# alessiodevoto/peekvit

Hardware: AMD Instinct MI355X
Metric: images/sec ViT-B/16 fwd @ batch 2048, 224x224 (higher is better)
Workload: dtype f16; 1 GPU; vit_b_16 forward, batch 2048/GPU, 224x224; global_batch=2048, parallelism=replicas x1 (batch-sharded, no collective), precision_mode=auto, streams=1, operands=IEEE fp16 operands, fp32 accumulate (same MFMA rate as bf16), range-guarded, range_guard_fallbacks=0

## Files before the change

peekvit_amd/_build.py:

```python
from __future__ import annotations

import glob
import os
import subprocess
import sys

HERE = os.path.dirname(os.path.abspath(__file__))
CSRC = os.path.join(HERE, "csrc")
LIB = os.path.join(HERE, "libpeekvit_hip.so")
LIB_F16 = os.path.join(HERE, "libpeekvit_hip_f16.so")
HIPCC = os.environ.get("HIPCC", "/opt/rocm/bin/hipcc")
FLAGS = ["--offload-arch=gfx950", "-O3", "-std=c++17", "-fPIC", "-Wno-unused-result"]
HEADERS = ("peekvit_hip.h", "peekvit_hip_moe.h", "peekvit_hip_ee.h", "peekvit_hip_sparse.h", "peekvit_hip_pct.h",
           "peekvit_hip_pct_train.h", "peekvit_hip_attn_stream.h", "peekvit_hip_pct_block.h", "peekvit_hip_rank_train.h", "peekvit_hip_rank_infer.h",
           "peekvit_hip_avit_train.h", "peekvit_hip_sparse_train.h", "peekvit_hip_avit_pack_train.h", "peekvit_hip_dropout.h", "peekvit_hip_sparse_long.h",
           "peekvit_hip_sparse_long_train.h", "peekvit_hip_avit_long.h")
FILE_FLAGS = {"pv_attention.hip": ["-mllvm", "-amdgpu-mfma-vgpr-form=1"], "pv_rowops.hip": ["-fno-slp-vectorize"],
              "pv_attention_stream.hip": ["-mllvm", "-amdgpu-mfma-vgpr-form=1"],
              "pv_ee.hip": ["-fno-slp-vectorize"],
              "pv_sparse.hip": ["-fno-slp-vectorize"],
              "pv_sparse_long.hip": ["-fno-slp-vectorize"],
              "pv_pct.hip": ["-fno-slp-vectorize"],
              "pv_pct_train.hip": ["-fno-slp-vectorize"],
              "pv_rank_train.hip": ["-fno-slp-vectorize"],
              "pv_avit_train.hip": ["-fno-slp-vectorize"],
              "pv_avit_pack_train.hip": ["-fno-slp-vectorize"],
              "pv_avit_long.hip": ["-fno-slp-vectorize"],
              "pv_dropout.hip": ["-fno-slp-vectorize"],
              "pv_sparse_train.hip": ["-fno-slp-vectorize", "-mllvm", "-amdgpu-mfma-vgpr-form=1"],
              "pv_sparse_long_train.hip": ["-fno-slp-vectorize"]}


def sources():
    return sorted(glob.glob(os.path.join(CSRC, "*.hip")))


def _stale() -> bool:
    if not os.path.exists(LIB) or not os.path.exists(LIB_F16):
        return True
    t = min(os.path.getmtime(LIB), os.path.getmtime(LIB_F16))
    deps = sources() + glob.glob(os.path.join(CSRC, "*.h")) + [os.path.join(os.path.dirname(HERE), "include", h) for h in HEADERS] + [os.path.abspath(__file__)]
    return any(os.path.getmtime(d) > t for d in deps)


def build(force: bool = False, verbose: bool = False) -> str:
    if not force and not _stale():
        return LIB
    procs = []
    variants = [("build", [], LIB), ("build_f16", ["-DPV_OPERAND_F16"], LIB_F16)]
# ... 49 lines not shown
```

peekvit_amd/_lib.py:

```python
from __future__ import annotations

import ctypes as C
import os
import threading

import torch

from ._build import LIB

_i64, _f32, _p, _i32 = C.c_int64, C.c_float, C.c_void_p, C.c_int32

PV_EPI_BIAS_BF16, PV_EPI_BIAS_GELU_BF16, PV_EPI_BIAS_RES_F32, PV_EPI_BIAS_POS_F32 = 0, 1, 2, 3
PV_EPI_BIAS_F32, PV_EPI_BIAS_GELU_SPLIT_BF16 = 4, 5
PV_EPI_BIAS_GELU_PAIR_BF16, PV_EPI_GELU_GRAD_BF16 = 6, 7
PV_WS_TRANSPOSE_COLSUM, PV_WS_COLSUM, PV_WS_LAYERNORM_BWD, PV_WS_GEMM_COLSUM_PARTIAL, PV_WS_GEMM_SPLITK = 1, 2, 3, 4, 5


class GemmArgs(C.Structure):
    _fields_ = [("struct_size", C.c_uint64), ("A", _p), ("W", _p), ("bias", _p), ("out", _p), ("res", _p), ("row_scale", _p), ("pos", _p),
                ("M", _i64), ("N", _i64), ("K", _i64), ("lda", _i64), ("ldw", _i64), ("ldo", _i64), ("ldr", _i64),
                ("rows_per_img_in", _i64), ("rows_per_img_out", _i64), ("row_off", _i64), ("qcols", _i64),
                ("qscale", _f32), ("epilogue", _i32),
                ("ln_gamma", _p), ("ln_beta", _p), ("ln_row_scale", _p), ("ln_out", _p), ("ln_eps", _f32),
                ("ksplit", _i32), ("colsum_partial", _p),
# ... 136 lines not shown

SIGNATURES_AVIT_PACK_TRAIN = {
    "pv_avit_pack_step_train": (C.c_int, [_p] * 4 + [_i64] * 4 + [_p] * 12 + [_i64, _p, _f32, _f32, _f32, C.c_int] + [_p] * 11),
    "pv_avit_pack_step_bwd": (C.c_int, [_p] * 16 + [_i64] * 6 + [_f32, C.c_int, _p]),
}

_u64 = C.c_uint64
SIGNATURES_DROPOUT = {
    "pv_dropout_keep_u8": (C.c_int, [_p, _u64, _u64, _i64, _i64, _f32, _p]),
    "pv_dropout_f32": (C.c_int, [_p, _p, _u64, _u64, _i64, _i64, _f32, _p]),
    "pv_dropout_residual": (C.c_int, [_p, _p, _p, _u64, _u64, _i64, _i64, _f32, _p]),
    "pv_dropout_bwd16": (C.c_int, [_p, _p, _u64, _u64, _i64, _i64, _f32, _p]),
    "pv_attention_stream_lse_drop_bf16": (C.c_int, [_p, _p, _p, _i64, _i64, _i64, _i64, _f32, _u64, _u64, _p, _p]),
    "pv_attention_stream_bwd16_drop_bf16": (C.c_int, [_p, _p, _p, _p, _p, _p, _p, _i64, _i64, _i64, _i64, _f32, _f32, _u64, _u64, _p]),
}

SIGNATURES_SPARSE_LONG = {
    "pv_attention_varlen_w_stream_bf16": SIGNATURES_SPARSE["pv_attention_varlen_w_bf16"],
    "pv_residual_pack_step_long": SIGNATURES_SPARSE["pv_residual_pack_step"],
}

SIGNATURES_SPARSE_LONG_TRAIN = {
    "pv_attention_varlen_w_stream_lse_bf16": SIGNATURES_SPARSE_TRAIN["pv_attention_varlen_w_lse_bf16"],
    "pv_attention_varlen_w_stream_bwd16_bf16": SIGNATURES_SPARSE_TRAIN["pv_attention_varlen_w_bwd16_bf16"],
    "pv_residual_pack_step_long_train": SIGNATURES_SPARSE_TRAIN["pv_residual_pack_step_train"],
    "pv_residual_pack_step_long_bwd": SIGNATURES_SPARSE_TRAIN["pv_residual_pack_step_bwd"],
}

SIGNATURES_AVIT_LONG = {
    "pv_avit_pack_step_long": SIGNATURES_AVIT_PACK_TRAIN["pv_avit_pack_step_train"],
    "pv_avit_pack_step_long_bwd": SIGNATURES_AVIT_PACK_TRAIN["pv_avit_pack_step_bwd"],
}

ABI_VERSION = 10
_lock = threading.Lock()
_libs: dict = {}

_OPERAND_DEFAULT = "bf16"
_tls = threading.local()
LIB_F16 = os.path.join(os.path.dirname(os.path.abspath(__file__)), "libpeekvit_hip_f16.so")


def current_operand() -> str:
    return getattr(_tls, "operand", _OPERAND_DEFAULT)


def set_operand(op: str) -> str:
    old = current_operand()
    _tls.operand = op
    return old


def __getattr__(name):
    if name == "OPERAND":
        return current_operand()
    raise AttributeError(f"module {__name__!r} has no attribute {name!r}")


def operand_dtype():
    import torch as _t
    return _t.float16 if current_operand() == "f16" else _t.bfloat16


class PeekvitHipError(RuntimeError):
    pass


def lib_path(operand: str = "bf16") -> str:
    return LIB_F16 if operand == "f16" else LIB


def load(operand=None):
    op = current_operand() if operand is None else operand
    lib = _libs.get(op)
    if lib is not None:
        return lib
    with _lock:
        lib = _libs.get(op)
        if lib is not None:
            return lib
        path = lib_path(op)
        if not os.path.exists(path):
            raise PeekvitHipError(
                f"{path} not found: the MI355X kernels are not built. Run `python -m peekvit_amd._build` "
                "(or __graft_entry__.build()); there is no fallback path.")
        lib = C.CDLL(path)
        for name, (res, args) in {**SIGNATURES, **SIGNATURES_MOE, **SIGNATURES_EE, **SIGNATURES_SPARSE, **SIGNATURES_PCT,
                                   **SIGNATURES_PCT_TRAIN, **SIGNATURES_ATTN_STREAM, **SIGNATURES_PCT_BLOCK, **SIGNATURES_RANK_TRAIN,
                                   **SIGNATURES_RANK_INFER, **SIGNATURES_AVIT_TRAIN, **SIGNATURES_SPARSE_TRAIN, **SIGNATURES_AVIT_PACK_TRAIN,
                                   **SIGNATURES_DROPOUT, **SIGNATURES_SPARSE_LONG, **SIGNATURES_SPARSE_LONG_TRAIN,
                                   **SIGNATURES_AVIT_LONG}.items():
            fn = getattr(lib, name)
            fn.restype, fn.argtypes = res, args
        if lib.pv_version() != ABI_VERSION:
            raise PeekvitHipError(f"{path} has ABI v{lib.pv_version()}, this package binds v{ABI_VERSION}: rebuild (python -m peekvit_amd._build)")
        if lib.pv_gemm_args_size() != C.sizeof(GemmArgs):
            raise PeekvitHipError(f"{path}: pv_gemm_args is {lib.pv_gemm_args_size()} bytes in the library, {C.sizeof(GemmArgs)} in this binding")
        if lib.pv_operand_type() != (1 if op == "f16" else 0):
            raise PeekvitHipError(f"{path} was built for a different operand type")
        _libs[op] = lib
    return lib


def check(code: int, what: str = "") -> None:
    if code != 0:
        msg = load().pv_error_string(code).decode()
        raise PeekvitHipError(f"{what}: {msg} (code {code})" if what else f"{msg} (code {code})")
```

peekvit_amd/csrc/pv_gemm.hip:

```cpp
#include "pv_rows.h"
#include "../../include/peekvit_hip_moe.h"
#include "pv_gelu_table.h"
#include <type_traits>
#include <cstdlib>

typedef __attribute__((ext_vector_type(8))) short s16x8;

#ifndef PV_STORE_NT
#define PV_STORE_NT 3
#endif
#define PV_STORE16(ptr, val) do { if (PV_STORE_NT & 1) __builtin_nontemporal_store((val), (ptr)); else *(ptr) = (val); } while (0)
#define PV_STORE32(ptr, val) do { if (PV_STORE_NT & 2) __builtin_nontemporal_store((val), (ptr)); else *(ptr) = (val); } while (0)
#ifndef PV_PF_MODE
#define PV_PF_MODE 2
#endif
#ifndef PV_EPI_PIPE
#define PV_EPI_PIPE 1
#endif

__device__ __forceinline__ float pv_fma_s(float a, float b, float c) {
    float r;
    asm("v_fma_f32 %0, %1, %2, %3" : "=v"(r) : "v"(a), "v"(b), "v"(c));
    return r;
}
__device__ __forceinline__ float pv_mul_s(float a, float b) {
    float r;
    asm("v_mul_f32 %0, %1, %2" : "=v"(r) : "v"(a), "v"(b));
    return r;
}
__device__ __forceinline__ float pv_gelu_poly(float x, const f32x4 c) {
    const pv_f32x2_t c02 = {c[0], c[1]}, c13 = {c[2], c[3]}, xx = {x, x};
    const pv_f32x2_t r = __builtin_elementwise_fma(c13, xx, c02);
    return pv_fma_s(x, pv_mul_s(x, r[1]), r[0]);
}
// ... 477 lines not shown
    if (row_off + Np > S || M > 0x7fffffff || B * S > 0x7fffffff) return PV_ERR_INVALID_ARG;
    GemmDev p = {};
    p.W = W; p.bias = bias; p.out = tokens; p.pos = pos;
    p.M = (int)M; p.N = (int)D; p.K = (int)(C * P * P);
    p.ldw = p.K; p.ldo = D;
    p.rpi = (int)Np; p.rpo = (int)S; p.row_off = (int)row_off;
    p.qscale = 1.0f;
    p.tiles_m = (int)((M + G1_BM - 1) / G1_BM); p.tiles_n = (int)((D + G1_BN - 1) / G1_BN);
    p.range_flag = range_flag;
    const PatchGeom gm = {img, (int)C, (int)R, (int)P, (int)Wp, (int)Np};
    static PvPerDevice attr_set;
    const int lds = 2 * 2 * G1_TILE_BYTES;
    if (attr_set.first_use()) (void)hipFuncSetAttribute(reinterpret_cast<const void*>(pv_patch_embed_kernel), hipFuncAttributeMaxDynamicSharedMemorySize, lds);
    PV_LAUNCH(pv_patch_embed_kernel, dim3((unsigned)(p.tiles_m * p.tiles_n)), dim3(256), lds, (hipStream_t)stream, p, gm);
    return pv_check_launch();
}

template <int EPI>
static int pv_launch_gemm128(const GemmDev& p, hipStream_t stream) {
    static PvPerDevice attr_set;
    const int lds = 2 * 2 * G1_TILE_BYTES;
    if (attr_set.first_use()) {
        (void)hipFuncSetAttribute(reinterpret_cast<const void*>(pv_gemm128_kernel<EPI>), hipFuncAttributeMaxDynamicSharedMemorySize, lds);
    }
    PV_LAUNCH(pv_gemm128_kernel<EPI>, dim3((unsigned)(p.tiles_m * p.tiles_n * (p.ksplit > 1 ? p.ksplit : 1))), dim3(256), lds, stream, p);
    return pv_check_launch();
}

constexpr int G2_BM = 256, G2_BN = 256, G2_BK = 64;
constexpr int G2_HALF = 128 * G2_BK * 2;
constexpr int G2_BUF = 4 * G2_HALF;
constexpr int G2_LDS = 2 * G2_BUF;

template <int EPI, bool PF = false, bool FULL = false, bool PERM = false>
__device__ __forceinline__ void pv_gemm256_tile(const GemmDev& p, char* smem, const int m0, const int n0, const bool first = true,
                                                const bool has_next = false, const int nm0 = 0, const int nn0 = 0, const int wid_pf = 0, const int slot_pf = 0) {
    int tid_ = threadIdx.x;
    if (PF) {
        int l_;
        asm volatile("v_mbcnt_lo_u32_b32 %0, -1, 0\n\tv_mbcnt_hi_u32_b32 %0, -1, %0" : "=v"(l_));
        tid_ = wid_pf * 64 + l_;
    }
    int tid = tid_, lane = tid & 63;
    const int wid = PF ? wid_pf : __builtin_amdgcn_readfirstlane(tid >> 6);
    const int wr = wid >> 2, wc = wid & 3;
#ifdef PV_STAMPS
    const size_t pv_stamp_slot = PF ? (size_t)slot_pf : (size_t)blockIdx.x;
#endif
    constexpr int PFM = PV_PF_MODE;
    constexpr int PF_BIAS_BASE = G2_LDS + ((EPI == PV_EPI_BIAS_GELU_BF16 || EPI == PV_EPI_BIAS_GELU_SPLIT_BF16 || EPI == PV_EPI_BIAS_GELU_PAIR_BF16) ? PV_GELU_CUB_N * PV_GELU_CUB_REP * 16 : 0) + 4096;
    PV_STAMP(14);
#ifdef PV_STAMPS
    if (threadIdx.x == 0 && p.dbg) { unsigned long long rt_; asm volatile("s_memrealtime %0\n\ts_waitcnt lgkmcnt(0)" : "=s"(rt_)::"memory"); p.dbg[pv_stamp_slot * 16 + 13] = rt_; }
#endif

    const int srow = wid * 8 + (lane >> 3);
    const int schunk = (lane & 7) ^ ((lane >> 3) & 7);
    const char* const a_blk = reinterpret_cast<const char*>(p.A + (int64_t)m0 * p.lda);
    const char* const w_blk = reinterpret_cast<const char*>(p.W + (int64_t)n0 * p.ldw);
    uint32_t oa[2][2], ow[2][2];
#pragma unroll
    for (int h = 0; h < 2; ++h)
#pragma unroll
        for (int j = 0; j < 2; ++j) {
            int ra = h * 128 + j * 64 + srow; ra = (FULL || m0 + ra < p.M) ? ra : p.M - 1 - m0;
            const int q = j * 64 + srow;
            int rw = h * 128 + (q & ~31) + (((q & 15) >> 2) << 3) + (((q >> 4) & 1) << 2) + (q & 3);
            rw = (FULL || n0 + rw < p.N) ? rw : p.N - 1 - n0;
            oa[h][j] = (uint32_t)(ra * (int)p.lda + schunk * 8) * 2u;
            ow[h][j] = (uint32_t)(rw * (int)p.ldw + schunk * 8) * 2u;
        }
    char* const lds_piece = smem + wid * 1024;
    auto stage_a = [&](int buf, int h, int kt) {
        const char* src = a_blk + kt * (G2_BK * 2);
        pv_glds16<PV_GEMM_A_AUX>(src + oa[h][0], lds_piece + buf * G2_BUF + h * G2_HALF);
        pv_glds16<PV_GEMM_A_AUX>(src + oa[h][1], lds_piece + buf * G2_BUF + h * G2_HALF + 8192);
    };
    auto stage_b = [&](int buf, int h, int kt) {
        const char* src = w_blk + kt * (G2_BK * 2);
        pv_glds16<PV_GEMM_W_AUX>(src + ow[h][0], lds_piece + buf * G2_BUF + (2 + h) * G2_HALF);
        pv_glds16<PV_GEMM_W_AUX>(src + ow[h][1], lds_piece + buf * G2_BUF + (2 + h) * G2_HALF + 8192);
    };
    auto stage_next_piece = [&](int tm0, int tn0, int pc) __attribute__((always_inline)) {
        if (pc == 8) {
            if (p.bias && wid < 4) {
                const int c_ = tn0 + wid * 64 + lane < p.N ? tn0 + wid * 64 + lane : p.N - 1;
                __builtin_amdgcn_global_load_lds((const __attribute__((address_space(1))) void*)(p.bias + c_),
                                                 (__attribute__((address_space(3))) void*)(smem + PF_BIAS_BASE + wid * 256), 4, 0, 0);
            }
            return;
        }
        const int h = (pc >> 1) & 1, jj = pc & 1;
        const int sr = wid * 8 + (lane >> 3), sc = (lane & 7) ^ ((lane >> 3) & 7);
        if (pc < 4) {
            const char* const na = reinterpret_cast<const char*>(p.A + (int64_t)tm0 * p.lda);
            int ra = h * 128 + jj * 64 + sr; ra = tm0 + ra < p.M ? ra : p.M - 1 - tm0;
            pv_glds16<PV_GEMM_A_AUX>(na + (uint32_t)(ra * (int)p.lda + sc * 8) * 2u, lds_piece + h * G2_HALF + jj * 8192);
        } else {
            const char* const nw = reinterpret_cast<const char*>(p.W + (int64_t)tn0 * p.ldw);
            const int q = jj * 64 + sr;
            int rw = h * 128 + (q & ~31) + (((q & 15) >> 2) << 3) + (((q >> 4) & 1) << 2) + (q & 3);
            rw = tn0 + rw < p.N ? rw : p.N - 1 - tn0;
            pv_glds16<PV_GEMM_W_AUX>(nw + (uint32_t)(rw * (int)p.ldw + sc * 8) * 2u, lds_piece + (2 + h) * G2_HALF + jj * 8192);
        }
    };

    typedef __attribute__((address_space(3))) const char lds_cc;
    const int frow = (lane & 15) * 128;
    const int fx0 = ((lane >> 4) ^ (lane & 7)) << 4;
    lds_cc* const lds0 = (lds_cc*)smem;
    lds_cc* a_rd[2][2];
    lds_cc* b_rd[2][2];
#pragma unroll
    for (int b = 0; b < 2; ++b)
#pragma unroll
// ... 9 lines not shown
    if (!PF) {
#pragma unroll
        for (int i = 0; i < 4; ++i) {
            f32x4 b4 = {0.f, 0.f, 0.f, 0.f};
            if (p.bias && en0 + (i >> 1) * 32 + (i & 1) * 4 < p.N) b4 = *reinterpret_cast<const f32x4*>(p.bias + en0 + (i >> 1) * 32 + (i & 1) * 4);
#pragma unroll
            for (int j = 0; j < 8; ++j) acc[i][j] = b4;
        }
    }
    bf16x8 af[2][4][2];
    bf16x8 bfr[2][2];

#define G2_READ_A(BUF, MH)                                                                                  \
    _Pragma("unroll") for (int t_ = 0; t_ < 4; ++t_) _Pragma("unroll") for (int ks_ = 0; ks_ < 2; ++ks_)  \
        af[MH][t_][ks_] = *reinterpret_cast<const __attribute__((address_space(3))) bf16x8*>(a_rd[BUF][ks_] + ((MH) * 4 + t_) * 2048);
#define G2_READ_B(BUF, NH)                                                                                  \
    _Pragma("unroll") for (int t_ = 0; t_ < 2; ++t_) _Pragma("unroll") for (int ks_ = 0; ks_ < 2; ++ks_)  \
        bfr[t_][ks_] = *reinterpret_cast<const __attribute__((address_space(3))) bf16x8*>(b_rd[BUF][ks_] + ((NH) * 2 + t_) * 2048);
#define G2_SYNC_LOADS()                                  \
    asm volatile("s_waitcnt lgkmcnt(0)" ::: "memory");   \
    __builtin_amdgcn_s_barrier();                        \
    __builtin_amdgcn_sched_barrier(0);
#define G2_MFMA(MH, NH)                                                                                              \
    __builtin_amdgcn_s_setprio(1);                                                                                   \
    _Pragma("unroll") for (int ks_ = 0; ks_ < 2; ++ks_) _Pragma("unroll") for (int n_ = 0; n_ < 2; ++n_)            \
        _Pragma("unroll") for (int m_ = 0; m_ < 4; ++m_)                                                            \
            acc[(NH) * 2 + n_][(MH) * 4 + m_] = PV_MFMA_16x16x32(                            \
                bfr[n_][ks_], af[MH][m_][ks_], acc[(NH) * 2 + n_][(MH) * 4 + m_], 0, 0, 0);                     \
    __builtin_amdgcn_s_setprio(0);                                                                                   \
    __builtin_amdgcn_sched_barrier(0);                                                                               \
    __builtin_amdgcn_s_barrier();                                                                                    \
    __builtin_amdgcn_sched_barrier(0);

    auto ktile = [&](auto buf_c, auto sb_c, auto sa_c, int kt) {
        constexpr int BUF = decltype(buf_c)::value;
        constexpr bool SB = decltype(sb_c)::value, SA = decltype(sa_c)::value;
        G2_READ_B(BUF, 0)
        __builtin_amdgcn_sched_barrier(0);
        G2_READ_A(BUF, 0)
        if (SB) stage_b(BUF ^ 1, 0, kt + 1);
        G2_SYNC_LOADS()
        G2_MFMA(0, 0)
        G2_READ_A(BUF, 1)
        if (SB) stage_b(BUF ^ 1, 1, kt + 1);
        G2_SYNC_LOADS()
        G2_MFMA(1, 0)
        G2_READ_B(BUF, 1)
        if (SA) stage_a(BUF, 0, kt + 2);
        G2_SYNC_LOADS()
        G2_MFMA(1, 1)
        if (SA) {
            stage_a(BUF, 1, kt + 2);
            asm volatile("s_waitcnt vmcnt(4)" ::: "memory");
        } else {
            asm volatile("s_waitcnt vmcnt(0)" ::: "memory");
        }
        G2_SYNC_LOADS()
        G2_MFMA(0, 1)
    };
    using B0 = std::integral_constant<int, 0>;
    using B1 = std::integral_constant<int, 1>;
    using T = std::true_type;
    using F = std::false_type;

    const int nk = p.K / G2_BK;
    if (PF) __builtin_assume(nk >= 4);
    PV_STAMP(0);
#ifdef PV_STAMPS
    if (threadIdx.x == 0 && p.dbg) { unsigned long long rt_; asm volatile("s_memrealtime %0\n\ts_waitcnt lgkmcnt(0)" : "=s"(rt_)::"memory"); p.dbg[pv_stamp_slot * 16 + 6] = rt_; }
#endif
    const bool own_tile0 = !PF || !PFM || first;
    if (PF && (first || !PFM) && p.bias && wid < 4) {
        const int c_ = n0 + wid * 64 + lane < p.N ? n0 + wid * 64 + lane : p.N - 1;
        __builtin_amdgcn_global_load_lds((const __attribute__((address_space(1))) void*)(p.bias + c_),
                                         (__attribute__((address_space(3))) void*)(smem + PF_BIAS_BASE + wid * 256), 4, 0, 0);
    }
    if (own_tile0) { stage_a(0, 0, 0); stage_a(0, 1, 0); stage_b(0, 0, 0); stage_b(0, 1, 0); }
    stage_a(1, 0, 1); stage_a(1, 1, 1);
    constexpr bool HAS_TAB = EPI == PV_EPI_BIAS_GELU_BF16 || EPI == PV_EPI_BIAS_GELU_SPLIT_BF16 || EPI == PV_EPI_BIAS_GELU_PAIR_BF16;
    constexpr int NTAB = HAS_TAB ? 2 : 0;
    if (HAS_TAB && own_tile0) {
#pragma unroll
        for (int i = 0; i < NTAB; ++i)
            pv_glds16(reinterpret_cast<const char*>(pv_gelu_cub) + (i * 512 + tid) * 16,
                      smem + G2_LDS + (i * 512 + wid * 64) * 16);
    }
    const bool fold_dma = PV_EPI_PIPE && (EPI == PV_EPI_BIAS_BF16 || EPI == PV_EPI_BIAS_GELU_BF16) && p.fold_stat != nullptr;
    if (fold_dma) {
        constexpr int FOLD_BASE = G2_LDS + (EPI == PV_EPI_BIAS_GELU_BF16 ? PV_GELU_CUB_N * PV_GELU_CUB_REP * 16 : 0);
        const int r_ = m0 + (tid >> 1) < p.M ? m0 + (tid >> 1) : p.M - 1;
        __builtin_amdgcn_global_load_lds((const __attribute__((address_space(1))) void*)(p.fold_stat + 2 * (int64_t)r_ + (tid & 1)),
                                         (__attribute__((address_space(3))) void*)(smem + FOLD_BASE + wid * 256), 4, 0, 0);
        const int c_ = n0 + (tid & 255) < p.N ? n0 + (tid & 255) : p.N - 1;
        __builtin_amdgcn_global_load_lds((const __attribute__((address_space(1))) void*)((tid < 256 ? p.fold_c1 : p.fold_c2) + c_),
                                         (__attribute__((address_space(3))) void*)(smem + FOLD_BASE + 2048 + wid * 256), 4, 0, 0);
    }
    if (own_tile0) {
        const int inflight = 4 + NTAB + (fold_dma ? 2 : 0);
        if (inflight == 4) asm volatile("s_waitcnt vmcnt(4)" ::: "memory");
        else if (inflight == 6) asm volatile("s_waitcnt vmcnt(6)" ::: "memory");
        else if (inflight == 8) asm volatile("s_waitcnt vmcnt(8)" ::: "memory");
        else asm volatile("s_waitcnt vmcnt(10)" ::: "memory");
        __builtin_amdgcn_s_barrier();
    }
    __builtin_amdgcn_sched_barrier(0);
    PV_STAMP(1);
    if (PF) {
#pragma unroll
        for (int i = 0; i < 4; ++i) {
            f32x4 b4 = {0.f, 0.f, 0.f, 0.f};
            if (p.bias) b4 = *reinterpret_cast<const __attribute__((address_space(3))) f32x4*>((const __attribute__((address_space(3))) char*)smem + PF_BIAS_BASE + (wc * 64 + ((lane >> 4) << 3) + (i >> 1) * 32 + (i & 1) * 4) * 4);
#pragma unroll
            for (int j = 0; j < 8; ++j) acc[i][j] = b4;
        }
    }
    if (wr == 1) __builtin_amdgcn_s_barrier();

    int kt = 0;
    for (; kt + 4 <= nk; kt += 2) {
        ktile(B0{}, T{}, T{}, kt);
        ktile(B1{}, T{}, T{}, kt + 1);
    }
    ktile(B0{}, T{}, F{}, kt);
    ktile(B1{}, F{}, F{}, kt + 1);
    if (wr == 0) __builtin_amdgcn_s_barrier();
    PV_STAMP(2);
#undef G2_READ_A
#undef G2_READ_B
#undef G2_SYNC_LOADS
#undef G2_MFMA

    typedef __attribute__((address_space(3))) char lds_c;
    lds_c* const cimg = (lds_c*)smem;
    if (PF) {
        asm volatile("v_mbcnt_lo_u32_b32 %0, -1, 0\n\tv_mbcnt_hi_u32_b32 %0, -1, %0" : "=v"(lane));
        tid = wid * 64 + lane;
        en0 = n0 + wc * 64 + ((lane >> 4) << 3);
    }
    const int g = lane >> 4, i16 = lane & 15;
    const bool pf_next = PF && PFM && has_next;
    if (PFM == 1 && pf_next) {
#pragma unroll
        for (int pc = 0; pc < 9; ++pc) stage_next_piece(nm0, nn0, pc);
    }
    if (PV_EPI_PIPE && (EPI == PV_EPI_BIAS_BF16 || EPI == PV_EPI_BIAS_GELU_BF16 || EPI == PV_EPI_BIAS_GELU_PAIR_BF16)) {
        float vmax = 0.f;
        const bool fold = p.fold_stat != nullptr;
        constexpr int FOLD_BASE = G2_LDS + (EPI != PV_EPI_BIAS_BF16 ? PV_GELU_CUB_N * PV_GELU_CUB_REP * 16 : 0);
        constexpr bool PAIR2 = EPI == PV_EPI_BIAS_GELU_PAIR_BF16;
        constexpr int NU = PAIR2 ? 32 : 16;
        if (fold) {
            f32x4 k1[2][2], k2[2][2];
#pragma unroll
            for (int u = 0; u < 2; ++u)
#pragma unroll
                for (int hh = 0; hh < 2; ++hh) {
                    const int col = wc * 64 + u * 32 + g * 8 + hh * 4;
                    k1[u][hh] = *reinterpret_cast<const __attribute__((address_space(3))) f32x4*>(cimg + FOLD_BASE + 2048 + col * 4);
                    k2[u][hh] = *reinterpret_cast<const __attribute__((address_space(3))) f32x4*>(cimg + FOLD_BASE + 3072 + col * 4);
// ... 459 lines not shown
}

template <int EPI>
__global__ __launch_bounds__(512) void pv_gemm256_pf_kernel(const GemmDev p) {
    extern __shared__ __attribute__((aligned(16))) char smem[];
    const int ntiles = p.tiles_m * p.tiles_n;
    const int xcd = blockIdx.x & 7, j = blockIdx.x >> 3, per = gridDim.x >> 3;
    const int q8 = ntiles >> 3, r8 = ntiles & 7;
    const int start = xcd < r8 ? xcd * (q8 + 1) : r8 * (q8 + 1) + (xcd - r8) * q8;
    const int cnt = q8 + (xcd < r8 ? 1 : 0);
    const int nfull = p.tiles_n / p.gc;
    auto decode = [&](int tile, int& m0, int& n0) {
        const int ch = min(tile / (p.gc * p.tiles_m), nfull);
        const int r = tile - ch * p.gc * p.tiles_m;
        const int cw = ch < nfull ? p.gc : p.tiles_n - nfull * p.gc;
        const int grp = r / (p.gm * cw), rem = r - grp * (p.gm * cw);
        const int gsz = min(p.gm, p.tiles_m - grp * p.gm);
        const int tnl = rem / gsz, tm = grp * p.gm + (rem - tnl * gsz);
        m0 = tm * G2_BM; n0 = (ch * p.gc + tnl) * G2_BN;
    };
    const int wid = __builtin_amdgcn_readfirstlane((int)threadIdx.x >> 6);
    int m0 = 0, n0 = 0, nm0 = 0, nn0 = 0;
    if (j < cnt) decode(start + j, m0, n0);
    for (int i = j; i < cnt; i += per) {
        const bool has_next = i + per < cnt;
        if (has_next) decode(start + i + per, nm0, nn0);
        if (m0 + G2_BM <= p.M && n0 + G2_BN <= p.N) pv_gemm256_tile<EPI, true, true>(p, smem, m0, n0, i == j, has_next, nm0, nn0, wid, start + i);
        else pv_gemm256_tile<EPI, true, false>(p, smem, m0, n0, i == j, has_next, nm0, nn0, wid, start + i);
        asm volatile("s_waitcnt lgkmcnt(0)" ::: "memory");
        __builtin_amdgcn_s_barrier();
        __builtin_amdgcn_sched_barrier(0);
        m0 = nm0; n0 = nn0;
    }
}

struct PvGroupDev {
    const int* tile_expert;
    int64_t w_stride;
    int E;
};

template <int EPI>
__global__ __launch_bounds__(512) void pv_gemm256_kernel(const GemmDev p_in, const PvGroupDev g) {
    extern __shared__ __attribute__((aligned(16))) char smem[];
    const int ntiles = p_in.tiles_m * p_in.tiles_n;
    const int tile = pv_xcd_remap(blockIdx.x, ntiles);
    const int tm = tile / p_in.tiles_n, tn = tile - tm * p_in.tiles_n;
    const int e = __builtin_amdgcn_readfirstlane(g.tile_expert[tm]);
    if (e < 0 || e >= g.E) return;
    GemmDev p = p_in;
    p.W += (int64_t)e * g.w_stride;
    if (p.bias) p.bias += (int64_t)e * p.N;
    const int m0 = tm * G2_BM, n0 = tn * G2_BN;
    constexpr bool PERM = EPI == PV_EPI_BIAS_RES_F32;
    if (n0 + G2_BN <= p.N) pv_gemm256_tile<EPI, false, true, PERM>(p, smem, m0, n0);
    else pv_gemm256_tile<EPI, false, false, PERM>(p, smem, m0, n0);
}

__global__ __launch_bounds__(512) void pv_gemm256_tn_kernel(const GemmDev p_in) {
    extern __shared__ __attribute__((aligned(16))) char smem[];
    GemmDev p = p_in;
    const int ntiles = p.tiles_m * p.tiles_n;
    int slice, tile;
    if (p.gm != 0) {
        const int l = pv_xcd_remap(blockIdx.x, ntiles * p.ksplit);
        slice = l / ntiles; tile = l - slice * ntiles;
// ... 932 lines not shown
```

peekvit_amd/engine.py:

```python
from __future__ import annotations

import math
import os
import threading
import warnings
import weakref
from typing import Dict, List, Optional, Tuple

import torch
from torch import nn

from . import _lib, autograph, ops
import contextlib

from ._lib import (PV_EPI_BIAS_BF16, PV_EPI_BIAS_F32, PV_EPI_BIAS_GELU_BF16, PV_EPI_BIAS_GELU_SPLIT_BF16, PV_EPI_BIAS_POS_F32,
                   PV_EPI_BIAS_RES_F32, PeekvitHipError)

_MODE_DEFAULT = os.environ.get("PEEKVIT_AMD_PRECISION", "auto")
_MODES = ("auto", "bf16", "f16", "bf16x3")
if _MODE_DEFAULT not in _MODES:
    raise ValueError(f"PEEKVIT_AMD_PRECISION={_MODE_DEFAULT!r}: expected one of {_MODES}")
_lib._OPERAND_DEFAULT = "f16" if _MODE_DEFAULT == "f16" else "bf16"
_mode_tls = threading.local()

# ... 1072 lines not shown
                                                             and nxt._pv_ranks_input()))
        x = call_module(layer, x)
        if x.is_inference() and _hooks_between(layer, nxt):
            for name in _HANDOFFS:
                if hasattr(x, name):
                    delattr(x, name)
    return x


_FUSED_PATCH_EMBED = os.environ.get("PEEKVIT_AMD_FUSED_PATCH_EMBED", "1") != "0"


def embed_tokens(model: nn.Module, img: torch.Tensor, budget_token: Optional[torch.Tensor] = None,
                 budget: float = 0.0) -> torch.Tensor:
    u8 = img.dtype == torch.uint8
    if not u8 and img.dtype != torch.float32:
        img = img.float()
    if not img.is_contiguous():
        img = img.contiguous()
    B = img.shape[0]
    P, D = model.patch_size, model.hidden_dim
    Hh, Ww, Cin = (img.shape[1], img.shape[2], img.shape[3]) if u8 else (img.shape[2], img.shape[3], img.shape[1])
    Np = (Hh // P) * (Ww // P)
    n_special = model.num_class_tokens + model.num_registers
    S = n_special + Np + (1 if budget_token is not None else 0)
    K = Cin * P * P
    dev = img.device

    if u8 and _mode() == "bf16x3":
        mt, st = norm_constants(model, img.device)
        img = ((img.permute(0, 3, 1, 2).float().div(255.0) - mt) / st).contiguous()
        u8 = False
    x3 = _mode() == "bf16x3" and not u8
    if _FUSED_PATCH_EMBED and not u8 and not x3 and D <= 512 and K % 64 == 0 and P % 8 == 0 and Hh == Ww and Hh % 4 == 0:
        tokens = torch.empty((B, S, D), dtype=torch.float32, device=dev)
        pos = _f32(model.encoder.pos_embedding).view(-1, D)
        ops.patch_embed(img, bf16_weight(model.conv_proj.weight).view(D, K), _f32(model.conv_proj.bias), pos, tokens, P, n_special)
        special = _f32(model.class_tokens).view(-1, D)
        if model.num_registers > 0:
            special = torch.cat([special, _f32(model.register_tokens).view(-1, D)], dim=0)
        ops.token_prologue(tokens, special, pos, _f32(budget_token), budget, n_special)
        return tokens
    cols = workspace.get("cols", (B * Np, 3 * K if x3 else K), _lib.operand_dtype(), dev)
    if x3:
        ops.im2col_split(img, P, cols)
    elif u8:
        mean, std = getattr(model, "input_mean", IMAGENET_MEAN), getattr(model, "input_std", IMAGENET_STD)
        ops.im2col_u8(img, P, cols, mean, std)
    else:
        ops.im2col(img, P, cols)
    tokens = torch.empty((B, S, D), dtype=torch.float32, device=dev)
    pos = _f32(model.encoder.pos_embedding).view(-1, D)
    wconv = (bf16x3_weight if x3 else bf16_weight)(model.conv_proj.weight)
    if K % 64 and not x3:
        Kp = (K + 63) // 64 * 64
        colsp = workspace.get("cols_pad", (B * Np, Kp), _lib.operand_dtype(), dev)
        colsp[:, K:].zero_()
        colsp[:, :K].copy_(cols)
        cols, wconv = colsp, _padded_k(model.conv_proj.weight, wconv, Kp)
    ops.gemm(cols, wconv, _f32(model.conv_proj.bias), tokens.view(B * S, D),
             PV_EPI_BIAS_POS_F32, M=B * Np, pos=pos, rows_per_img_in=Np, rows_per_img_out=S, row_off=n_special)
    special = _f32(model.class_tokens).view(-1, D)
    if model.num_registers > 0:
        special = torch.cat([special, _f32(model.register_tokens).view(-1, D)], dim=0)
    ops.token_prologue(tokens, special, pos, _f32(budget_token), budget, n_special)
    return tokens


_wpadcache: Dict[tuple, tuple] = {}

# ... 775 lines not shown
```

peekvit_amd/ops.py:

```python
from __future__ import annotations

import ctypes as C
from typing import Optional

import torch

from . import _lib
from ._lib import GemmArgs, check

launch_count = 0


class KernelTimer:

    def __init__(self):
        self.records = []

    def __enter__(self):
        global _timer
        _timer = self
        return self

    def __exit__(self, *exc):
        global _timer
# ... 107 lines not shown
        raise _lib.PeekvitHipError(f"{name}: expected a GPU tensor, got {t.device}")
    if t.dtype != dtype:
        raise _lib.PeekvitHipError(f"{name}: expected {dtype}, got {t.dtype}")
    if not t.is_contiguous():
        raise _lib.PeekvitHipError(f"{name}: expected a contiguous tensor")
    return t


def _count():
    global launch_count
    launch_count += 1


def cast_bf16(src: torch.Tensor, out: Optional[torch.Tensor] = None) -> torch.Tensor:
    _chk(src, torch.float32, "src")
    if out is None:
        out = torch.empty(src.shape, dtype=_lib.operand_dtype(), device=src.device)
    with _timed("pv_cast_f32_bf16", src.device, 0.0, 6.0 * src.numel()):
        check(_lib.load().pv_cast_f32_bf16(_ptr(src), _ptr(out), src.numel(), _stream(src)), "pv_cast_f32_bf16")
    _count()
    return out


def patch_embed(x: torch.Tensor, w: torch.Tensor, bias: Optional[torch.Tensor], pos: torch.Tensor, tokens: torch.Tensor, patch: int, row_off: int) -> torch.Tensor:
    _chk(x, torch.float32, "x"); _chk(w, _lib.operand_dtype(), "w"); _chk(pos, torch.float32, "pos"); _chk(tokens, torch.float32, "tokens")
    B, Cc, H, W = x.shape
    _, S, D = tokens.shape
    if H != W or w.shape != (D, Cc * patch * patch) or pos.shape[1] != D or pos.shape[0] < row_off + (H // patch) ** 2:
        raise _lib.PeekvitHipError(f"patch_embed: shapes x {tuple(x.shape)}, w {tuple(w.shape)}, pos {tuple(pos.shape)}, tokens {tuple(tokens.shape)}")
    M = B * (H // patch) ** 2
    with _timed("pv_gemm_bf16", x.device, 2.0 * M * D * w.shape[1], 4.0 * x.numel() + 2.0 * w.numel() + 4.0 * M * D, member=(D, w.shape[1], _lib.PV_EPI_BIAS_POS_F32)):
        check(_lib.load().pv_patch_embed_f32(_ptr(x), _ptr(w), _ptr(bias), _ptr(pos), _ptr(tokens), B, Cc, H, patch, D, S, row_off, _flag(x.device), _stream(x)),
              "pv_patch_embed_f32")
    _count()
    return tokens


def im2col(x: torch.Tensor, patch: int, out: torch.Tensor) -> torch.Tensor:
    _chk(x, torch.float32, "x")
    B, Cc, H, W = x.shape
    with _timed("pv_im2col_bf16", x.device, 0.0, 6.0 * x.numel()):
        check(_lib.load().pv_im2col_bf16(_ptr(x), _ptr(out), B, Cc, H, W, patch, _flag(x.device), _stream(x)), "pv_im2col_bf16")
    _count()
    return out


def im2col_u8(x: torch.Tensor, patch: int, out: torch.Tensor, mean, std) -> torch.Tensor:
    _chk(x, torch.uint8, "x")
    B, H, W, Cc = x.shape
    if Cc != 3:
        raise _lib.PeekvitHipError("uint8 input must be NHWC with 3 channels")
    with _timed("pv_im2col_u8_bf16", x.device, 0.0, 3.0 * x.numel()):
        check(_lib.load().pv_im2col_u8_bf16(_ptr(x), _ptr(out), B, H, W, patch, *[float(v) for v in mean], *[float(v) for v in std],
                                            _stream(x)), "pv_im2col_u8_bf16")
    _count()
    return out


def token_prologue(tokens, special, pos, budget_token, budget: float, n_special: int):
    B, S, D = tokens.shape
    with _timed("pv_token_prologue", tokens.device, 0.0, 0.0):
        check(_lib.load().pv_token_prologue(_ptr(tokens), _ptr(special), _ptr(pos), _ptr(budget_token), float(budget),
                                            B, S, D, n_special, _stream(tokens)), "pv_token_prologue")
    _count()


# ... 1648 lines not shown
```

Measured before the change: 27300 images/sec.

## Fuse patch im2col gather into 256-tile GEMM for wide patch embedding

```diff
diff --git a/include/peekvit_hip_patch256.h b/include/peekvit_hip_patch256.h
--- /dev/null
+++ b/include/peekvit_hip_patch256.h
@@ -0,0 +1,16 @@
+#ifndef PEEKVIT_HIP_PATCH256_H
+#define PEEKVIT_HIP_PATCH256_H
+
+#include "peekvit_hip.h"
+
+#ifdef __cplusplus
+extern "C" {
+#endif
+
+int pv_patch_embed256_f32(const float* img, const uint16_t* W, const float* bias, const float* pos, float* tokens, int64_t B, int64_t C, int64_t R,
+                          int64_t P, int64_t D, int64_t S, int64_t row_off, uint32_t* range_flag, void* stream);
+
+#ifdef __cplusplus
+}
+#endif
+#endif
diff --git a/peekvit_amd/_build.py b/peekvit_amd/_build.py
--- a/peekvit_amd/_build.py
+++ b/peekvit_amd/_build.py
@@ -14,7 +14,7 @@
 HEADERS = ("peekvit_hip.h", "peekvit_hip_moe.h", "peekvit_hip_ee.h", "peekvit_hip_sparse.h", "peekvit_hip_pct.h",
            "peekvit_hip_pct_train.h", "peekvit_hip_attn_stream.h", "peekvit_hip_pct_block.h", "peekvit_hip_rank_train.h", "peekvit_hip_rank_infer.h",
            "peekvit_hip_avit_train.h", "peekvit_hip_sparse_train.h", "peekvit_hip_avit_pack_train.h", "peekvit_hip_dropout.h", "peekvit_hip_sparse_long.h",
-           "peekvit_hip_sparse_long_train.h", "peekvit_hip_avit_long.h")
+           "peekvit_hip_sparse_long_train.h", "peekvit_hip_avit_long.h", "peekvit_hip_patch256.h")
 FILE_FLAGS = {"pv_attention.hip": ["-mllvm", "-amdgpu-mfma-vgpr-form=1"], "pv_rowops.hip": ["-fno-slp-vectorize"],
               "pv_attention_stream.hip": ["-mllvm", "-amdgpu-mfma-vgpr-form=1"],
               "pv_ee.hip": ["-fno-slp-vectorize"],
diff --git a/peekvit_amd/_lib.py b/peekvit_amd/_lib.py
--- a/peekvit_amd/_lib.py
+++ b/peekvit_amd/_lib.py
@@ -192,6 +192,10 @@
     "pv_avit_pack_step_long_bwd": SIGNATURES_AVIT_PACK_TRAIN["pv_avit_pack_step_bwd"],
 }
 
+SIGNATURES_PATCH256 = {
+    "pv_patch_embed256_f32": SIGNATURES["pv_patch_embed_f32"],
+}
+
 ABI_VERSION = 10
 _lock = threading.Lock()
 _libs: dict = {}
@@ -249,7 +253,7 @@
                                    **SIGNATURES_PCT_TRAIN, **SIGNATURES_ATTN_STREAM, **SIGNATURES_PCT_BLOCK, **SIGNATURES_RANK_TRAIN,
                                    **SIGNATURES_RANK_INFER, **SIGNATURES_AVIT_TRAIN, **SIGNATURES_SPARSE_TRAIN, **SIGNATURES_AVIT_PACK_TRAIN,
                                    **SIGNATURES_DROPOUT, **SIGNATURES_SPARSE_LONG, **SIGNATURES_SPARSE_LONG_TRAIN,
-                                   **SIGNATURES_AVIT_LONG}.items():
+                                   **SIGNATURES_AVIT_LONG, **SIGNATURES_PATCH256}.items():
             fn = getattr(lib, name)
             fn.restype, fn.argtypes = res, args
         if lib.pv_version() != ABI_VERSION:
diff --git a/peekvit_amd/csrc/pv_gemm.hip b/peekvit_amd/csrc/pv_gemm.hip
--- a/peekvit_amd/csrc/pv_gemm.hip
+++ b/peekvit_amd/csrc/pv_gemm.hip
@@ -1,5 +1,6 @@
 #include "pv_rows.h"
 #include "../../include/peekvit_hip_moe.h"
+#include "../../include/peekvit_hip_patch256.h"
 #include "pv_gelu_table.h"
 #include <type_traits>
 #include <cstdlib>
@@ -543,9 +544,11 @@
 constexpr int G2_BUF = 4 * G2_HALF;
 constexpr int G2_LDS = 2 * G2_BUF;
 
-template <int EPI, bool PF = false, bool FULL = false, bool PERM = false>
+template <int EPI, bool PF = false, bool FULL = false, bool PERM = false, bool GATHER = false>
 __device__ __forceinline__ void pv_gemm256_tile(const GemmDev& p, char* smem, const int m0, const int n0, const bool first = true,
-                                                const bool has_next = false, const int nm0 = 0, const int nn0 = 0, const int wid_pf = 0, const int slot_pf = 0) {
+                                                const bool has_next = false, const int nm0 = 0, const int nn0 = 0, const int wid_pf = 0, const int slot_pf = 0,
+                                                const PatchGeom* const gm = nullptr) {
+    static_assert(!GATHER || (EPI == PV_EPI_BIAS_POS_F32 && FULL && !PF && !PERM), "the patch gather exists for full tiles of the one-tile stem launch only");
     int tid_ = threadIdx.x;
     if (PF) {
         int l_;
@@ -592,6 +595,54 @@
         pv_glds16<PV_GEMM_W_AUX>(src + ow[h][0], lds_piece + buf * G2_BUF + (2 + h) * G2_HALF);
         pv_glds16<PV_GEMM_W_AUX>(src + ow[h][1], lds_piece + buf * G2_BUF + (2 + h) * G2_HALF + 8192);
     };
+    const char* px_base = nullptr;
+    uint32_t px_off[2][2] = {};
+    float px_invp = 0.f;
+    f32x4 px[2][2][2];
+    float px_vmax = 0.f;
+    uint32_t px_lds = 0;
+    if constexpr (GATHER) {
+        const int b0 = m0 / gm->Np;
+        px_base = reinterpret_cast<const char*>(gm->img + (int64_t)b0 * gm->C * gm->R * gm->R);
+        px_invp = 1.0f / (float)gm->P;
+#pragma unroll
+        for (int h = 0; h < 2; ++h)
+#pragma unroll
+            for (int j = 0; j < 2; ++j) {
+                const int ra = m0 + h * 128 + j * 64 + srow;
+                const int b = ra / gm->Np, pi = ra - b * gm->Np, py = pi / gm->Wp, pxx = pi - py * gm->Wp;
+                px_off[h][j] = (uint32_t)((((b - b0) * gm->C * gm->R + py * gm->P) * gm->R + pxx * gm->P) * 4);
+            }
+        px_lds = (uint32_t)(uintptr_t)((__attribute__((address_space(3))) char*)smem) + (uint32_t)(wid * 1024 + lane * 16);
+    }
+    auto px_koff = [&](int kt) -> uint32_t {
+        const int k = kt * G2_BK + schunk * 8, P_ = gm->P;
+        const int q = (int)(((float)k + 0.5f) * px_invp), kx = k - q * P_;
+        const int c = (int)(((float)q + 0.5f) * px_invp), ky = q - c * P_;
+        return (uint32_t)(((c * gm->R + ky) * gm->R + kx) * 4);
+    };
+    auto px_fetch = [&](f32x4 (&dst)[2][2], int rs, int kt) __attribute__((always_inline)) {
+        const uint32_t ko = px_koff(kt);
+#pragma unroll
+        for (int h = 0; h < 2; ++h) {
+            const uint32_t vo = px_off[h][rs] + ko;
+            asm volatile("global_load_dwordx4 %0, %1, %2" : "=&v"(dst[h][0]) : "v"(vo), "s"(px_base) : "memory");
+            asm volatile("global_load_dwordx4 %0, %1, %2 offset:16" : "=&v"(dst[h][1]) : "v"(vo), "s"(px_base) : "memory");
+        }
+    };
+    auto px_wait = [&](f32x4 (&r)[2][2], auto n_c) __attribute__((always_inline)) {
+        asm volatile("s_waitcnt vmcnt(%4)" : "+v"(r[0][0]), "+v"(r[0][1]), "+v"(r[1][0]), "+v"(r[1][1]) : "n"(decltype(n_c)::value) : "memory");
+    };
+    auto px_put = [&](const f32x4 (&src)[2][2], int buf, int rs) __attribute__((always_inline)) {
+#pragma unroll
+        for (int h = 0; h < 2; ++h) {
+            const u32x4 v = {pv_pack_bf16x2_tracked(src[h][0][0], src[h][0][1], px_vmax), pv_pack_bf16x2_tracked(src[h][0][2], src[h][0][3], px_vmax),
+                             pv_pack_bf16x2_tracked(src[h][1][0], src[h][1][1], px_vmax), pv_pack_bf16x2_tracked(src[h][1][2], src[h][1][3], px_vmax)};
+            asm volatile("ds_write_b128 %0, %1" ::"v"(px_lds + (uint32_t)(buf * G2_BUF + h * G2_HALF + rs * 8192)), "v"(v) : "memory");
+        }
+    };
+    using PxN6 = std::integral_constant<int, 6>;
+    using PxN8 = std::integral_constant<int, 8>;
     auto stage_next_piece = [&](int tm0, int tn0, int pc) __attribute__((always_inline)) {
         if (pc == 8) {
             if (p.bias && wid < 4) {
@@ -667,13 +718,17 @@
     __builtin_amdgcn_s_barrier();                                                                                    \
     __builtin_amdgcn_sched_barrier(0);
 
-    auto ktile = [&](auto buf_c, auto sb_c, auto sa_c, int kt) {
+    auto ktile = [&](auto buf_c, auto sb_c, auto sa_c, int kt, const bool f1) {
         constexpr int BUF = decltype(buf_c)::value;
         constexpr bool SB = decltype(sb_c)::value, SA = decltype(sa_c)::value;
         G2_READ_B(BUF, 0)
         __builtin_amdgcn_sched_barrier(0);
         G2_READ_A(BUF, 0)
         if (SB) stage_b(BUF ^ 1, 0, kt + 1);
+        if constexpr (GATHER) {
+            if (SB) { px_wait(px[0], PxN6{}); px_put(px[0], BUF ^ 1, 0); }
+            if (SA) px_fetch(px[0], 0, kt + 2);
+        }
         G2_SYNC_LOADS()
         G2_MFMA(0, 0)
         G2_READ_A(BUF, 1)
@@ -681,11 +736,15 @@
         G2_SYNC_LOADS()
         G2_MFMA(1, 0)
         G2_READ_B(BUF, 1)
-        if (SA) stage_a(BUF, 0, kt + 2);
+        if constexpr (GATHER) {
+            if (SA) { px_wait(px[1], PxN8{}); px_put(px[1], BUF, 1); }
+            if (SA && f1) px_fetch(px[1], 1, kt + 3);
+        } else if (SA) stage_a(BUF, 0, kt + 2);
         G2_SYNC_LOADS()
         G2_MFMA(1, 1)
-        if (SA) {
-            stage_a(BUF, 1, kt + 2);
+        if constexpr (GATHER) { G2_READ_A(BUF, 0) }
+        if (SA && (!GATHER || f1)) {
+            if constexpr (!GATHER) stage_a(BUF, 1, kt + 2);
             asm volatile("s_waitcnt vmcnt(4)" ::: "memory");
         } else {
             asm volatile("s_waitcnt vmcnt(0)" ::: "memory");
@@ -699,7 +758,7 @@
     using F = std::false_type;
 
     const int nk = p.K / G2_BK;
-    if (PF) __builtin_assume(nk >= 4);
+    if (PF || GATHER) __builtin_assume(nk >= 4);
     PV_STAMP(0);
 #ifdef PV_STAMPS
     if (threadIdx.x == 0 && p.dbg) { unsigned long long rt_; asm volatile("s_memrealtime %0\n\ts_waitcnt lgkmcnt(0)" : "=s"(rt_)::"memory"); p.dbg[pv_stamp_slot * 16 + 6] = rt_; }
@@ -710,8 +769,26 @@
         __builtin_amdgcn_global_load_lds((const __attribute__((address_space(1))) void*)(p.bias + c_),
                                          (__attribute__((address_space(3))) void*)(smem + PF_BIAS_BASE + wid * 256), 4, 0, 0);
     }
+    if constexpr (GATHER) {
+        stage_b(0, 0, 0); stage_b(0, 1, 0);
+        f32x4 pa[3][2][2];
+#pragma unroll
+        for (int s = 0; s < 3; ++s) px_fetch(pa[s], s == 0 ? 0 : 1, s >> 1);
+        px_fetch(px[0], 0, 1);
+        px_fetch(px[1], 1, 2);
+        asm volatile("s_waitcnt vmcnt(0)"
+                     : "+v"(pa[0][0][0]), "+v"(pa[0][0][1]), "+v"(pa[0][1][0]), "+v"(pa[0][1][1]), "+v"(pa[1][0][0]), "+v"(pa[1][0][1]), "+v"(pa[1][1][0]),
+                       "+v"(pa[1][1][1]), "+v"(pa[2][0][0]), "+v"(pa[2][0][1]), "+v"(pa[2][1][0]), "+v"(pa[2][1][1]), "+v"(px[0][0][0]), "+v"(px[0][0][1]),
+                       "+v"(px[0][1][0]), "+v"(px[0][1][1]), "+v"(px[1][0][0]), "+v"(px[1][0][1]), "+v"(px[1][1][0]), "+v"(px[1][1][1])
+                     :: "memory");
+#pragma unroll
+        for (int s = 0; s < 3; ++s) px_put(pa[s], s >> 1, s == 0 ? 0 : 1);
+        asm volatile("s_waitcnt lgkmcnt(0)" ::: "memory");
+        __builtin_amdgcn_s_barrier();
+    } else {
     if (own_tile0) { stage_a(0, 0, 0); stage_a(0, 1, 0); stage_b(0, 0, 0); stage_b(0, 1, 0); }
     stage_a(1, 0, 1); stage_a(1, 1, 1);
+    }
     constexpr bool HAS_TAB = EPI == PV_EPI_BIAS_GELU_BF16 || EPI == PV_EPI_BIAS_GELU_SPLIT_BF16 || EPI == PV_EPI_BIAS_GELU_PAIR_BF16;
     constexpr int NTAB = HAS_TAB ? 2 : 0;
     if (HAS_TAB && own_tile0) {
@@ -730,7 +807,7 @@
         __builtin_amdgcn_global_load_lds((const __attribute__((address_space(1))) void*)((tid < 256 ? p.fold_c1 : p.fold_c2) + c_),
                                          (__attribute__((address_space(3))) void*)(smem + FOLD_BASE + 2048 + wid * 256), 4, 0, 0);
     }
-    if (own_tile0) {
+    if (!GATHER && own_tile0) {
         const int inflight = 4 + NTAB + (fold_dma ? 2 : 0);
         if (inflight == 4) asm volatile("s_waitcnt vmcnt(4)" ::: "memory");
         else if (inflight == 6) asm volatile("s_waitcnt vmcnt(6)" ::: "memory");
@@ -753,13 +830,14 @@
 
     int kt = 0;
     for (; kt + 4 <= nk; kt += 2) {
-        ktile(B0{}, T{}, T{}, kt);
-        ktile(B1{}, T{}, T{}, kt + 1);
-    }
-    ktile(B0{}, T{}, F{}, kt);
-    ktile(B1{}, F{}, F{}, kt + 1);
+        ktile(B0{}, T{}, T{}, kt, true);
+        ktile(B1{}, T{}, T{}, kt + 1, kt + 4 < nk);
+    }
+    ktile(B0{}, T{}, F{}, kt, false);
+    ktile(B1{}, F{}, F{}, kt + 1, false);
     if (wr == 0) __builtin_amdgcn_s_barrier();
     PV_STAMP(2);
+    if constexpr (GATHER) pv_range_commit(px_vmax, p.range_flag);
 #undef G2_READ_A
 #undef G2_READ_B
 #undef G2_SYNC_LOADS
@@ -1285,6 +1363,43 @@
         __builtin_amdgcn_sched_barrier(0);
         m0 = nm0; n0 = nn0;
     }
+}
+
+__global__ __launch_bounds__(512) void pv_stem256_kernel(const GemmDev p, const PatchGeom gm) {
+    extern __shared__ __attribute__((aligned(16))) char smem[];
+    const int tile = pv_xcd_remap(blockIdx.x, p.tiles_m * p.tiles_n);
+    const int tm = tile / p.tiles_n, tn = tile - tm * p.tiles_n;
+    pv_gemm256_tile<PV_EPI_BIAS_POS_F32, false, true, false, true>(p, smem, tm * G2_BM, tn * G2_BN, true, false, 0, 0, 0, 0, &gm);
+}
+
+extern "C" int pv_patch_embed256_f32(const float* img, const uint16_t* W, const float* bias, const float* pos, float* tokens, int64_t B, int64_t C, int64_t R,
+                                     int64_t P, int64_t D, int64_t S, int64_t row_off, uint32_t* range_flag, void* stream) {
+    if (!img || !W || !pos || !tokens || B <= 0 || C <= 0 || R <= 0 || P <= 0 || D <= 0 || S <= 0 || row_off < 0 || ((uintptr_t)range_flag & 3)) return PV_ERR_INVALID_ARG;
+    if (R % P || P % 8 || (C * P * P) % (2 * G2_BK) || D % G2_BN || ((uintptr_t)img & 15) || ((uintptr_t)W & 15) || ((uintptr_t)tokens & 15) || ((uintptr_t)pos & 15) ||
+        (bias && ((uintptr_t)bias & 15)))
+        return PV_ERR_UNSUPPORTED;
+    const int64_t Wp = R / P, Np = Wp * Wp, M = B * Np, K = C * P * P;
+    if (M % G2_BM || K < 4 * G2_BK) return PV_ERR_UNSUPPORTED;
+    if (row_off + Np > S) return PV_ERR_INVALID_ARG;
+    if (M > 0x7fffffff || B * S > 0x7fffffff || K > 65536 || D > 0x7fffffff || ((255 + Np - 1) / Np + 1) * C * R * R * 4 > 0x7fffffffLL) return PV_ERR_UNSUPPORTED;
+    if ((M / G2_BM) * (D / G2_BN) > 0x7fffffff) return PV_ERR_UNSUPPORTED;
+    GemmDev p = {};
+    p.W = W; p.bias = bias; p.out = tokens; p.pos = pos;
+    p.M = (int)M; p.N = (int)D; p.K = (int)K;
+    p.ldw = K; p.ldo = D;
+    p.rpi = (int)Np; p.rpo = (int)S; p.row_off = (int)row_off;
+    p.qscale = 1.0f;
+    p.tiles_m = (int)(M / G2_BM); p.tiles_n = (int)(D / G2_BN);
+    p.gm = 1; p.gc = p.tiles_n;
+    p.range_flag = range_flag;
+#ifdef PV_STAMPS
+    p.dbg = g_pv_dbg;
+#endif
+    const PatchGeom gm = {img, (int)C, (int)R, (int)P, (int)Wp, (int)Np};
+    static PvPerDevice attr_set;
+    if (attr_set.first_use()) (void)hipFuncSetAttribute(reinterpret_cast<const void*>(pv_stem256_kernel), hipFuncAttributeMaxDynamicSharedMemorySize, G2_LDS);
+    PV_LAUNCH(pv_stem256_kernel, dim3((unsigned)(p.tiles_m * p.tiles_n)), dim3(512), G2_LDS, (hipStream_t)stream, p, gm);
+    return pv_check_launch();
 }
 
 struct PvGroupDev {
diff --git a/peekvit_amd/engine.py b/peekvit_amd/engine.py
--- a/peekvit_amd/engine.py
+++ b/peekvit_amd/engine.py
@@ -1128,10 +1128,12 @@
         img = ((img.permute(0, 3, 1, 2).float().div(255.0) - mt) / st).contiguous()
         u8 = False
     x3 = _mode() == "bf16x3" and not u8
-    if _FUSED_PATCH_EMBED and not u8 and not x3 and D <= 512 and K % 64 == 0 and P % 8 == 0 and Hh == Ww and Hh % 4 == 0:
+    wide = (_FUSED_PATCH_EMBED and not u8 and not x3 and D > 512 and Hh == Ww and ops.patch_embed256_supported(B, Cin, Hh, P, D)
+            and (B * Np // 256) * (D // 256) >= 128)
+    if wide or (_FUSED_PATCH_EMBED and not u8 and not x3 and D <= 512 and K % 64 == 0 and P % 8 == 0 and Hh == Ww and Hh % 4 == 0):
         tokens = torch.empty((B, S, D), dtype=torch.float32, device=dev)
         pos = _f32(model.encoder.pos_embedding).view(-1, D)
-        ops.patch_embed(img, bf16_weight(model.conv_proj.weight).view(D, K), _f32(model.conv_proj.bias), pos, tokens, P, n_special)
+        (ops.patch_embed256 if wide else ops.patch_embed)(img, bf16_weight(model.conv_proj.weight).view(D, K), _f32(model.conv_proj.bias), pos, tokens, P, n_special)
         special = _f32(model.class_tokens).view(-1, D)
         if model.num_registers > 0:
             special = torch.cat([special, _f32(model.register_tokens).view(-1, D)], dim=0)
diff --git a/peekvit_amd/ops.py b/peekvit_amd/ops.py
--- a/peekvit_amd/ops.py
+++ b/peekvit_amd/ops.py
@@ -163,6 +163,27 @@
     with _timed("pv_gemm_bf16", x.device, 2.0 * M * D * w.shape[1], 4.0 * x.numel() + 2.0 * w.numel() + 4.0 * M * D, member=(D, w.shape[1], _lib.PV_EPI_BIAS_POS_F32)):
         check(_lib.load().pv_patch_embed_f32(_ptr(x), _ptr(w), _ptr(bias), _ptr(pos), _ptr(tokens), B, Cc, H, patch, D, S, row_off, _flag(x.device), _stream(x)),
               "pv_patch_embed_f32")
+    _count()
+    return tokens
+
+
+def patch_embed256_supported(B: int, Cc: int, R: int, patch: int, D: int) -> bool:
+    if patch <= 0 or R % patch or patch % 8:
+        return False
+    K, M = Cc * patch * patch, B * (R // patch) ** 2
+    return K % 128 == 0 and 256 <= K <= 65536 and D % 256 == 0 and M % 256 == 0
+
+
+def patch_embed256(x: torch.Tensor, w: torch.Tensor, bias: Optional[torch.Tensor], pos: torch.Tensor, tokens: torch.Tensor, patch: int, row_off: int) -> torch.Tensor:
+    _chk(x, torch.float32, "x"); _chk(w, _lib.operand_dtype(), "w"); _chk(pos, torch.float32, "pos"); _chk(tokens, torch.float32, "tokens")
+    B, Cc, H, W = x.shape
+    _, S, D = tokens.shape
+    if H != W or w.shape != (D, Cc * patch * patch) or pos.shape[1] != D or pos.shape[0] < row_off + (H // patch) ** 2 or tokens.shape[0] != B:
+        raise _lib.PeekvitHipError(f"patch_embed256: shapes x {tuple(x.shape)}, w {tuple(w.shape)}, pos {tuple(pos.shape)}, tokens {tuple(tokens.shape)}")
+    M = B * (H // patch) ** 2
+    with _timed("pv_patch_embed256_f32", x.device, 2.0 * M * D * w.shape[1], 4.0 * x.numel() + 4.0 * M * D + 2.0 * w.numel()):
+        check(_lib.load().pv_patch_embed256_f32(_ptr(x), _ptr(w), _ptr(bias), _ptr(pos), _ptr(tokens), B, Cc, H, patch, D, S, row_off, _flag(x.device), _stream(x)),
+              "pv_patch_embed256_f32")
     _count()
     return tokens
 
```

After: 27330 images/sec, median of 2. No clear change (+0.1%).
